# jinhan/tacotron2-vae

Hardware: AMD Instinct MI355X
Metric: mel-frames/s (train step, batch=6, 80-mel) (higher is better)
Workload: dtype f32; 1 GPU; configs[1]: Tacotron2-VAE fp32 train step (fwd+loss+bwd+clip+Adam), B=6/GPU fixed shape T_in=84 T_out=400, dropout on, random-init seed 1234; step_mode=hip-graph replay, decoder_forward=persistent, decoder_backward=persistent, startup_steps=43, global_batch=6, parallelism=dp1

## Files before the change

include/t2vae.h:

```cpp
#ifndef T2VAE_H
#define T2VAE_H
#include <stdint.h>
#ifdef __cplusplus
extern "C" {
#endif

#define T2V_OK 0
#define T2V_ERR_DIMS -1
#define T2V_ERR_ARG -2
#define T2V_ERR_LAUNCH -3

const char* t2v_version(void);
const char* t2v_last_error(void);

void t2v_set_phase_profile(unsigned long long* dev_buf32);
int t2v_stamp(unsigned long long* dev_buf, int slot, void* stream);
int t2v_debug_spin(int wgs, int microseconds, void* stream);

typedef struct t2v_step_params {
    uint64_t epoch;
    float lr;
    float bc1;
    float bc2s;
    float kl_weight;
// ... 224 lines not shown
int t2v_decoder_infer_steps_window(const t2v_dec_weights* w, const t2v_dec_infer_bufs* s, int B, int T_in,
                                   int t_begin, int t_end, float gate_threshold, float p_prenet,
                                   int external_prenet, uint64_t seed, const t2v_dec_items* items,
                                   const t2v_dec_window* window, void* stream);
int t2v_decoder_infer_persistent_window(const t2v_dec_persist_weights* w, const t2v_dec_persist_bufs* s, int B, int T_in,
                                        int t_end, float gate_threshold, float p_prenet, uint64_t seed,
                                        const t2v_dec_items* items, const t2v_dec_window* window, void* stream);

int t2v_decoder_infer_steps_plan(const t2v_dec_weights* w, const t2v_dec_infer_bufs* s, int B, int T_in,
                                 int t_begin, int t_end, float gate_threshold, float p_prenet,
                                 int external_prenet, uint64_t seed, const t2v_dec_items* items,
                                 const t2v_dec_window* window, const int32_t* plan, int plan_stride, const int32_t* n_plan,
                                 void* stream);
int t2v_decoder_infer_persistent_plan(const t2v_dec_persist_weights* w, const t2v_dec_persist_bufs* s, int B, int T_in,
                                      int t_end, float gate_threshold, float p_prenet, uint64_t seed,
                                      const t2v_dec_items* items, const t2v_dec_window* window, const int32_t* plan,
                                      int plan_stride, const int32_t* n_plan, void* stream);

#define T2V_PLAN_MAX_SYMBOLS 4096
int t2v_duration_plan(const float* dur, int dur_stride, const int32_t* n_ids, const float* rate, int rate_stride_b,
                      int rate_stride_j, int B, int S, int T_max, int32_t* plan, int plan_stride, int32_t* n_plan,
                      void* stream);

int t2v_conv1d_stat_blocks(int B, int T, int Cin, int Cout, int KS);
int t2v_conv1d_stat_blocks_bf16(int B, int T, int Cin, int Cout, int KS);
long long t2v_conv1d_staged_launches(void);
int t2v_conv1d_fwd(const float* W, const float* X, const float* bias, float* Y, float* stat_part,
                   int B, int Cin, int T, int Cout, int KS, void* stream);
int t2v_conv1d_dw_scratch_floats(int B, int Cin, int T, int Cout, int KS);
int t2v_conv1d_bwd(const float* W, const float* X, const float* dY, float* dX, float* dW, float* Wt_scratch,
                   float* dw_scratch,
                   int B, int Cin, int T, int Cout, int KS, void* stream);
int t2v_conv1d_flip_weights(const float* const* W, float* const* Wt, const int* Cout, const int* Cin, int KS, int n,
                            void* stream);
int t2v_conv1d_fwd_bf16(const float* W, const float* X, const float* bias, float* Y, float* stat_part,
                        void* Wp_scratch, int B, int Cin, int T, int Cout, int KS, void* stream);
int t2v_conv1d_bwd_bf16(const float* W, const float* X, const float* dY, float* dX, float* dW,
                        void* Wp_scratch, float* dw_scratch, int B, int Cin, int T, int Cout, int KS, void* stream);

int t2v_bn_act_fwd(const float* y, const float* stat_part, int nblk, const float* gamma, const float* beta,
                   float* running_mean, float* running_var, float* mean_out, float* rstd_out, float* out,
                   int B, int M, int T, int act, int training, float p_drop, float momentum, float eps,
                   uint64_t seed, uint32_t rng_stream, uint32_t rng_t, void* stream);
int t2v_bn_act_fwd_len(const float* y, const float* gamma, const float* beta, const float* running_mean,
                       const float* running_var, float* out, const int32_t* lengths, int B, int M, int T, int act, float eps,
                       void* stream);
int t2v_bn_act_bwd(const float* y, const float* dout, const float* mean, const float* rstd,
                   const float* gamma, const float* beta, float* dy, float* dgamma, float* dbeta,
                   float* dconv_bias, int B, int M, int T, int act, float p_drop, uint64_t seed,
                   uint32_t rng_stream, uint32_t rng_t, void* stream);
int t2v_bn_act_bwd_eval(const float* y, const float* dout, const float* mean, const float* rstd,
                   const float* gamma, const float* beta, float* dy, float* dgamma, float* dbeta,
                   float* dconv_bias, int B, int M, int T, int act, float p_drop, uint64_t seed,
                   uint32_t rng_stream, uint32_t rng_t, void* stream);
int t2v_bn_act_slices(int backward, int B, int M, int T, int training, int has_partials);

int t2v_embedding_fwd(const long long* ids, const float* W, float* out_bct, int B, int T, int C, int n_symbols, void* stream);
int t2v_embedding_bwd(const long long* ids, const float* dy_bct, float* dW, int B, int T, int C, int n_symbols, void* stream);

int t2v_gemm_epilogue_bwd(const float* dy, const float* y, float* out, size_t n, float scale, void* stream);

long t2v_colsum_scratch_floats(long M, long N);
int t2v_colsum(const float* A, long lda, long M, long N, float* scratch, float* out, void* stream);

int t2v_mask_outputs(float* mel, float* mel_post, float* gate, const int* lengths, int B, int C, int T, float gate_fill,
                     void* stream);
int t2v_mask_time(const float* x, float* out, const int32_t* lengths, int B, int C, int T, void* stream);
int t2v_reparam_fwd(const float* eps, const float* mu, const float* logvar, float* z, long n, void* stream);
int t2v_reparam_bwd(const float* dz, const float* eps, const float* logvar, float* dlogvar, long n, void* stream);
int t2v_gather_words(const void* const* src, void* const* dst, int n, void* stream);
int t2v_concat2_rows(const float* a, long lda, int na, const float* b, long ldb, int nb, float* out, long rows, void* stream);

int t2v_bilstm_fwd(const float* gx, const float* whh, const int32_t* lengths, float* y, float* gates,
                   float* cells, float* hx_scratch, uint32_t* sync3, int B, int T, void* stream);
int t2v_bilstm_bwd(const float* whh, const int32_t* lengths, const float* dy, const float* gates,
                   const float* cells, float* dg, float* dgx_scratch, uint32_t* sync3, int B, int T,
                   void* stream);

int t2v_gemm_f32(const float* A, long sAi, long sAk, const float* B, long sBj, long sBk, const float* bias,
                 float* C, int ldc, int M, int N, int K, int relu, int accumulate, float p_drop,
                 uint64_t seed, uint32_t rng_stream, uint32_t rng_t, void* stream);
long t2v_gemm_splitk_scratch_floats(int M, int N, int K);
int t2v_gemm_f32_splitk(const float* A, long sAi, long sAk, const float* B, long sBj, long sBk, const float* bias,
                        float* C, int ldc, int M, int N, int K, int relu, int accumulate, float p_drop,
                        uint64_t seed, uint32_t rng_stream, uint32_t rng_t, float* splitk_scratch, void* stream);

int t2v_gemm_f32_set_mode(int x3);

typedef struct t2v_gemm_group {
    const float* A;
    long sAi;
    long sAk;
    int nb;
    const float* B[3];
    long sBj[3];
    long sBk[3];
    int N[3];
    float* C[3];
    int ldc[3];
} t2v_gemm_group;
long t2v_gemm_f32_grouped_scratch_floats(const t2v_gemm_group* groups, int ngroups, int M, int K);
int t2v_gemm_f32_grouped(const t2v_gemm_group* groups, int ngroups, int M, int K, int accumulate, float* scratch, void* stream);
long t2v_gemm_f32_grouped_group_offset(const t2v_gemm_group* groups, int ngroups, int M, int K, int g);
int t2v_gemm_f32_grouped_handed(const t2v_gemm_group* groups, int ngroups, int M, int K, int accumulate, float* scratch, int handed,
                                const uint32_t* done_ctr, int done_cap, void* stream);
long t2v_gemm_bf16_grouped_scratch_floats(const t2v_gemm_group* groups, int ngroups, int M, int K);
int t2v_gemm_bf16_grouped(const t2v_gemm_group* groups, int ngroups, int M, int K, int accumulate, float* scratch, void* stream);

int t2v_conv1d_x3_set_mode(int mode);
int t2v_conv1d_takes_x3(int B, int Cin, int T, int Cout, int KS, int bf16);
#define T2V_CONV_OP_FWD 0
#define T2V_CONV_OP_DX 1
#define T2V_CONV_OP_DW 2
#define T2V_CONV_ROUTE_GEMM 0
#define T2V_CONV_ROUTE_FWD 1
#define T2V_CONV_ROUTE_FWD_DMA 2
#define T2V_CONV_ROUTE_X3 3
#define T2V_CONV_ROUTE_BF16 4
#define T2V_CONV_ROUTE_BF16K32 5
#define T2V_CONV_ROUTE_PLANE1 6
#define T2V_CONV_ROUTE_DW 7
#define T2V_CONV_ROUTE_DW_BF16 8
#define T2V_CONV_ROUTES 9
int t2v_conv1d_route(int op, int B, int Cin, int T, int Cout, int KS, int bf16, int w_mod16, int* fallback, int* tile, int* ksplit,
                     int* dw_splits, int* stat_blocks, int* dw_scratch_floats, int* plane_splits, int* plane_chunk);
const char* t2v_conv1d_route_name(int route);

int t2v_gemm_f32_batched(const float* A, long sAb, long sAi, long sAk, const float* B, long sBb, long sBj, long sBk,
                         float* C, long sCb, int ldc, int nbatch, int M, int N, int K, void* stream);
int t2v_gemm_bf16(const float* A, long sAi, long sAk, const float* B, long sBj, long sBk, const float* bias,
                  float* C, int ldc, int M, int N, int K, int relu, int accumulate, float p_drop,
                  uint64_t seed, uint32_t rng_stream, uint32_t rng_t, void* stream);
long t2v_gemm_bf16_splitk_scratch_floats(int M, int N, int K);
int t2v_gemm_bf16_splitk(const float* A, long sAi, long sAk, const float* B, long sBj, long sBk, const float* bias,
                         float* C, int ldc, int M, int N, int K, int relu, int accumulate, float p_drop,
                         uint64_t seed, uint32_t rng_stream, uint32_t rng_t, float* splitk_scratch, void* stream);

#define T2V_GEMM_ROUTE_F32_64 0
#define T2V_GEMM_ROUTE_F32_64_SPLITK 1
#define T2V_GEMM_ROUTE_F32_BIG_128 2
#define T2V_GEMM_ROUTE_F32_BIG_64 3
#define T2V_GEMM_ROUTE_F32_X3 4
#define T2V_GEMM_ROUTE_BF16_64 5
#define T2V_GEMM_ROUTE_BF16_64_SPLITK 6
#define T2V_GEMM_ROUTE_BF16_BIG 7
#define T2V_GEMM_ROUTE_BF16_BIG_SPLITK 8
#define T2V_GEMM_ROUTE_BF16_PLANES 9
#define T2V_GEMM_ROUTE_BF16_TO_F32_BIG 10
#define T2V_GEMM_ROUTES 11
int t2v_gemm_route(int M, int N, int K, long sAi, long sAk, long sBj, long sBk, int a_mod16, int b_mod16, int scratch_mod16,
                   int has_scratch, int relu, float p_drop, int bf16, int* form, int* splits, int* k_per_split);
const char* t2v_gemm_route_name(int route);


int t2v_conv2d_s2_fwd(const float* x, const float* w, const float* bias, float* y, int B, int Cx, int H, int W,
                      int Cout, int coord, void* stream);
int t2v_conv2d_s2_dw_scratch_floats(int B, int Cx, int H, int W, int Cout, int coord);
int t2v_conv2d_s2_bwd(const float* x, const float* w, const float* dy, float* dx, float* dw, float* dw_scratch,
                      int B, int Cx, int H, int W, int Cout, int coord, void* stream);

long t2v_conv2d_s2_gemm_scratch_floats(int B, int Cx, int H, int W, int Cout, int coord);
int t2v_conv2d_s2_fwd_gemm(const float* x, const float* w, const float* bias, float* y, float* scratch, int B, int Cx, int H, int W,
                           int Cout, int coord, void* stream);
int t2v_conv2d_s2_bwd_gemm(const float* x, const float* w, const float* dy, float* dx, float* dw, float* scratch, int B, int Cx, int H,
                           int W, int Cout, int coord, void* stream);
int t2v_gru_fwd(const float* gi, const float* whh, const float* bhh, float* hs, float* gsave, float* xchg,
                uint32_t* sync2, int B, int T, void* stream);
int t2v_gru_bwd(const float* whh, const float* hs, const float* gsave, const float* dh_last, float* dgi,
                float* dgh, float* xchg, uint32_t* sync2, int B, int T, void* stream);

int t2v_conv2d_s2_fwd_ragged(const float* x, const float* w, const float* bias, float* y, const int32_t* hlen, int B, int Cx,
                             int H, int W, int Cout, int coord, int x_tstride, void* stream);
long t2v_conv2d_s2_gemm_ragged_scratch_floats(int B, int Cx, int H, int W, int Cout, int coord);
int t2v_conv2d_s2_fwd_gemm_ragged(const float* x, const float* w, const float* bias, float* y, float* scratch,
                                  const int32_t* hlen, int B, int Cx, int H, int W, int Cout, int coord, int x_tstride,
                                  void* stream);
int t2v_gru_fwd_len(const float* gi, const float* whh, const float* bhh, float* hs, float* gsave, float* xchg,
                    uint32_t* sync2, const int32_t* steps, float* h_last, int B, int T, void* stream);
int t2v_loss_fwd_bwd(const float* mel, const float* post, const float* mel_t, const float* gate,
                     const float* gate_t, const float* mu, const float* logvar, float* dmel, float* dpost,
                     float* dgate, float* dmu, float* dlogvar, float* part192, float* out4, uint32_t* ticket,
                     uint64_t n_mel, int n_gate, int n_lat, float kl_weight, void* stream);

int t2v_clip_adam_step(float* params, float* grads, float* exp_avg, float* exp_avg_sq, uint64_t n,
                       float lr, float beta1, float beta2, float eps, float weight_decay,
                       float max_norm, float inv_world, float bc1, float bc2, float* partials,
                       float* norm_out, void* stream);
int t2v_clip_adam_step_guarded(float* params, float* grads, float* exp_avg, float* exp_avg_sq, uint64_t n,
                               float lr, float beta1, float beta2, float eps, float weight_decay,
                               float max_norm, float inv_world, float bc1, float bc2, float* partials,
                               float* norm_out, const uint32_t* guard, int guard_n, void* stream);
int t2v_clip_adam_ema_step_guarded(float* params, float* grads, float* exp_avg, float* exp_avg_sq, uint64_t n,
                                   float lr, float beta1, float beta2, float eps, float weight_decay,
                                   float max_norm, float inv_world, float bc1, float bc2, float* partials,
                                   float* norm_out, const uint32_t* guard, int guard_n, float* ema, float ema_rate,
                                   int ema_warmup, uint64_t ema_t, void* stream);

int t2v_mel_frontend(const float* wav_f32, const int16_t* wav_i16, const int64_t* n_samples, int B,
                     int n_stride, float scale, int n_fft, int hop, int n_mel, const float* window,
                     const float* tw512, const float* tw1024, const int32_t* mel_start,
                     const int32_t* mel_len, const float* mel_w, int maxw, float* mel_out,
                     int t_stride, void* stream);

int t2v_stft_polar(const float* wav, const int64_t* n_samples, int B, int n_stride, int n_fft, int hop,
                   const float* window, const float* tw512, const float* tw1024, float* mag, float* phase,
                   int t_stride, void* stream);
size_t t2v_istft_scratch_bytes(int B, int t_stride);
int t2v_istft(const float* mag, const float* phase, const int32_t* n_frames, int B, int t_stride, int n_fft, int hop,
              const float* window, const float* tw512, const float* tw1024, void* scratch, float* out, int out_stride,
              void* stream);
size_t t2v_griffin_lim_scratch_bytes(int B, int t_stride);
int t2v_griffin_lim(const float* mag, const float* angles, const int32_t* n_frames, int B, int t_stride, int n_fft,
                    int hop, int n_iters, const float* window, const float* tw512, const float* tw1024, void* scratch,
                    float* out, int out_stride, void* stream);
int t2v_mel_to_magnitude(const float* mel, const float* pinv_basis, const int32_t* n_frames, int B, int t_stride,
                         int n_mel, float* mag, void* stream);
size_t t2v_griffin_lim_fast_scratch_bytes(int B, int t_stride);
int t2v_griffin_lim_fast(const float* mag, const float* angles, const int32_t* n_frames, int B, int t_stride, int n_fft,
                         int hop, int n_iters, float momentum, const float* window, const float* tw512,
                         const float* tw1024, void* scratch, float* out, int out_stride, void* stream);
int t2v_mel_to_magnitude_nnls(const float* mel, const float* pinv_basis, const int32_t* tap_lo, const float* tap_w0,
                              const float* tap_w1, const int32_t* filt_start, const int32_t* filt_len, float lipschitz,
                              int n_iters, const int32_t* n_frames, int B, int t_stride, int n_mel, float* mag,
                              void* stream);

#define T2V_DTW_MAX_FRAMES 2048
size_t t2v_mel_dtw_scratch_bytes(int B, int tx_max, int ty_max);
int t2v_mel_dtw(const float* X, const int32_t* nx, int x_stride, const float* Y, const int32_t* ny, int y_stride,
                int B, int n_mel, float* dist, void* scratch, void* stream);

#define T2V_TSNE_MAX_POINTS 16384
#define T2V_TSNE_EXAG_ITERS 250
size_t t2v_tsne_scratch_bytes(int N, int D);
int t2v_tsne_affinities(const float* X, int N, int D, float perplexity, float* P, void* scratch, void* stream);
int t2v_tsne_gradient(const float* P, const float* Y, int N, float exaggeration, float* grad, float* kl_or_null,
                      void* scratch, void* stream);
int t2v_tsne_run(const float* P, float* Y_inout, int N, int n_iter, float learning_rate, float* kl_trace, void* scratch,
                 void* stream);

#define T2V_F0_MAX_LAG 400
int t2v_f0_yin(const float* y, const int32_t* n, int y_stride, int B, int tau_min, int tau_max, float threshold, float* f0,
               float* aperiodicity, int out_stride, void* stream);

#define T2V_ALIGN_FRAMES 16
size_t t2v_alignment_scratch_bytes(int B, int N, int T_in);
int t2v_alignment_stats(const float* A, long long a_stride_b, long long a_stride_t, const int32_t* n_frames,
                        const int32_t* n_text, int B, int N, int T_in, int max_jump, float cover_min, int32_t* path,
                        int path_stride, float* mass, int mass_stride, float* focus, int32_t* stats, void* scratch,
                        void* stream);

#define T2V_RESAMPLE_MAX_TAPS 32768
int t2v_resample(const void* x, int x_is_pcm16, float scale, const int32_t* n, int x_stride, int B, const float* taps, int up,
                 int down, int half, float* y, int out_stride, void* stream);
int t2v_trim_bounds(const float* y, const int32_t* n, int y_stride, int B, float top_db, int pad_frames, float* ms, int ms_stride,
                    int32_t* bounds, void* stream);
int t2v_crop_rows(const float* y, int y_stride, const int32_t* bounds, int B, void* out, int out_is_pcm16, int out_stride,
                  int32_t* stats, void* stream);

#define T2V_LATENT_MAX_POINTS 16384
#define T2V_LATENT_MAX_CLASSES 8
#define T2V_LATENT_MAX_K 32
#define T2V_LATENT_TILE 128
size_t t2v_latent_scratch_bytes(int N, int M, int C, int k, int slice_rows);
int t2v_latent_neighbours(const float* R, const int32_t* labels, int N, int D, int C, const float* Q, int M,
                          const int32_t* exclude, const int32_t* target, int k, int slice_rows, int32_t* nn_idx,
                          float* nn_dist, float* class_sum, int32_t* class_cnt, int32_t* rank, void* scratch, void* stream);

#define T2V_NCEP 13
#define T2V_ALIGNED_COUNTS 4
#define T2V_ALIGNED_SUMS 8
int t2v_mel_cepstrum(const float* M, const int32_t* n, int m_stride, int B, int n_mel, int n_cep, const float* table, float* out,
                     int out_stride, void* stream);
size_t t2v_cep_dtw_scratch_bytes(int B, int tx_max, int ty_max);
int t2v_cep_dtw_forward(const float* X, const int32_t* nx, int x_stride, const float* Y, const int32_t* ny, int y_stride, int B,
                        int n_cep, float* dist, void* scratch, void* stream);
int t2v_cep_dtw_walk(const int32_t* nx, int x_stride, const int32_t* ny, int y_stride, int B, const void* scratch, int32_t* K,
                     int32_t* path, int path_stride, void* stream);
int t2v_cep_dtw_path(const float* X, const int32_t* nx, int x_stride, const float* Y, const int32_t* ny, int y_stride, int B,
                     int n_cep, float* dist, int32_t* K, int32_t* path, int path_stride, void* scratch, void* stream);
int t2v_path_scores(const int32_t* path, const int32_t* K, int path_stride, const float* X, const int32_t* nx, int x_stride,
                    const float* Y, const int32_t* ny, int y_stride, const float* fx, int fx_stride, const float* fy, int fy_stride,
                    int B, int n_cep, int32_t* counts, float* sums, void* stream);

#define T2V_LOUDNESS_CHUNK 64
#define T2V_LOUDNESS_TILE 16384
size_t t2v_loudness_scratch_bytes(int B, int y_stride, int hop);
int t2v_loudness(const float* y, const int32_t* n, int y_stride, int B, const double* table, int hop, float* frame_ms,
                 int ms_stride, float* block_pw, int blk_stride, int32_t* rows, void* scratch, void* stream);
int t2v_scale_rows(float* y, const int32_t* n, int y_stride, int B, const float* gains, void* stream);

#define T2V_TSM_BINS 513
#define T2V_TSM_MAX_RATIO 1023
#define T2V_TSM_MAX_FRAMES (1 << 20)
size_t t2v_phase_vocoder_scratch_bytes(int B, int out_stride, int phase_lock);
int t2v_phase_vocoder(const float* mag, const float* phase, const int32_t* n_frames, int B, int T, int t_stride, int num, int den,
                      int phase_lock, float* mag_out, float* phase_out, int out_stride, void* scratch, void* stream);

size_t t2v_spsi_scratch_bytes(int B, int t_stride);
int t2v_spsi(const float* mag, const int32_t* n_frames, int B, int T, int t_stride, float* phase_out, void* scratch, void* stream);

#define T2V_ENV_BINS 513
#define T2V_ENV_MAX_ORDER 256
#define T2V_ENV_MAX_ITERS 32
int t2v_spectral_envelope(const float* mag, const int32_t* n_frames, int B, int T, int t_stride, int order, int iters, int p, int q,
                          float* log_env_out, float* mag_out, int out_stride, void* stream);

// ... 25 lines not shown
```

tacotron2-vae_amd/csrc/gemm.hip:

```cpp
#include <stdlib.h>
#include <string.h>
#include "t2v_common.h"
#include "t2v_kernels.h"
#include "t2v_coop.h"
#include "t2v_x3.h"
#include "t2v_xchg.h"
#include "gemm_x3_tile.h"

#define GM_BM 64
#define GM_BN 64
#define GM_BK 32

struct GemmArgs {
    const float* A; const float* B; const float* bias; float* C;
    long sAi, sAk, sBj, sBk;
    int M, N, K, ldc;
    int relu, accumulate;
    float p_drop; uint64_t seed; uint32_t rng_stream, rng_t;
    const t2v_step_params* step;
    int kz_chunk;
    float* part;
    int nbatch;
    long sAb, sBb, sCb;
    int nsub;
    long sAs, sBs;
    int bias_row;
    unsigned* tile_ctr;
};

__device__ __forceinline__ void gemm64_epilogue(const GemmArgs& a, f32x16& acc, int i0, int j0, int wm, int wn, int lane, int tid) {
    const int j = j0 + 32 * wn + (lane & 31);
    if (a.part) {
        if (j < a.N) {
#pragma unroll
            for (int r = 0; r < 16; ++r) {
                const int i = i0 + 32 * wm + (r & 3) + 8 * (r >> 2) + 4 * (lane >> 5);
                if (i < a.M) st_sc1(a.part + ((size_t)blockIdx.z * a.M + i) * a.N + j, acc[r]);
            }
        }
        __shared__ unsigned last_;
        asm volatile("s_waitcnt vmcnt(0)" ::: "memory");
        __syncthreads();
        unsigned* ctr = a.tile_ctr + blockIdx.y * gridDim.x + blockIdx.x;
        if (tid == 0) last_ = __hip_atomic_fetch_add(ctr, 1u, __ATOMIC_RELAXED, __HIP_MEMORY_SCOPE_AGENT) == gridDim.z - 1 ? 1u : 0u;
        __syncthreads();
        if (!last_) return;
        if (tid == 0) __hip_atomic_store(ctr, 0u, __ATOMIC_RELAXED, __HIP_MEMORY_SCOPE_AGENT);
        const int nz = (int)gridDim.z;
#pragma unroll
        for (int r = 0; r < 16; ++r) acc[r] = 0.f;
        if (j < a.N) {
            for (int z0 = 0; z0 < nz; z0 += 4) {
                float v[4][16];
#pragma unroll
                for (int u = 0; u < 4; ++u) {
                    const int z = min(z0 + u, nz - 1);
#pragma unroll
                    for (int r = 0; r < 16; ++r) {
                        const int i = min(i0 + 32 * wm + (r & 3) + 8 * (r >> 2) + 4 * (lane >> 5), a.M - 1);
                        v[u][r] = ld_sc1(a.part + ((size_t)z * a.M + i) * a.N + j);
                    }
                }
#pragma unroll
                for (int u = 0; u < 4; ++u)
                    if (z0 + u < nz) {
#pragma unroll
                        for (int r = 0; r < 16; ++r) acc[r] += v[u][r];
                    }
            }
        }
    }
    if (j < a.N) {
        const float bv = (a.bias && !a.bias_row) ? a.bias[j] : 0.f;
#pragma unroll
        for (int r = 0; r < 16; ++r) {
            const int i = i0 + 32 * wm + (r & 3) + 8 * (r >> 2) + 4 * (lane >> 5);
            if (i < a.M) {
                const size_t idx = (size_t)i * a.ldc + j;
                float v = acc[r] + ((a.bias && a.bias_row) ? a.bias[i] : bv);
                if (a.accumulate) v += a.C[idx];
                if (a.relu) v = fmaxf(v, 0.f);
                if (a.p_drop > 0.f) v *= t2v_drop_scale(t2v_step_seed(a.seed, a.step), a.rng_stream, a.rng_t, (uint32_t)idx, a.p_drop);
                a.C[idx] = v;
            }
        }
    }
}

template <bool A_KC, bool B_KC>
__global__ __launch_bounds__(256) void k_gemm_f32(GemmArgs a) {
    __shared__ float As[2][GM_BK][GM_BM + 1];
    __shared__ float Bs[2][GM_BK][GM_BN + 1];
    const int tid = threadIdx.x, wave = tid >> 6, lane = tid & 63;
    const int wm = wave >> 1, wn = wave & 1;
    const int i0 = blockIdx.y * GM_BM, j0 = blockIdx.x * GM_BN;
    if (a.nbatch > 1) {
        const int zb = a.nsub > 1 ? blockIdx.z / a.nsub : blockIdx.z, zs = a.nsub > 1 ? blockIdx.z - zb * a.nsub : 0;
        a.A += zb * a.sAb + zs * a.sAs; a.B += zb * a.sBb + zs * a.sBs; a.C += blockIdx.z * a.sCb;
    }
    const int kbeg = a.kz_chunk ? blockIdx.z * a.kz_chunk : 0, kend = a.kz_chunk ? min(a.K, kbeg + a.kz_chunk) : a.K;
    constexpr int NE = GM_BM * GM_BK / 256;
    float ra[NE], rb[NE];
    auto load_tiles = [&](int k0) {
#pragma unroll
        for (int e8 = 0; e8 < NE; ++e8) {
            const int e = tid + 256 * e8;
            {
                const int kk = A_KC ? (e & (GM_BK - 1)) : (e >> 6);
                const int ii = A_KC ? (e >> 5) : (e & (GM_BM - 1));
                const int i = i0 + ii, k = k0 + kk;
                ra[e8] = (i < a.M && k < kend) ? a.A[(long)i * a.sAi + (long)k * a.sAk] : 0.f;
            }
            {
                const int kk = B_KC ? (e & (GM_BK - 1)) : (e >> 6);
                const int jj = B_KC ? (e >> 5) : (e & (GM_BN - 1));
                const int j = j0 + jj, k = k0 + kk;
                rb[e8] = (j < a.N && k < kend) ? a.B[(long)j * a.sBj + (long)k * a.sBk] : 0.f;
            }
        }
    };
    auto store_tiles = [&](int buf) {
#pragma unroll
        for (int e8 = 0; e8 < NE; ++e8) {
            const int e = tid + 256 * e8;
            if (A_KC) As[buf][e & (GM_BK - 1)][e >> 5] = ra[e8]; else As[buf][e >> 6][e & (GM_BM - 1)] = ra[e8];
            if (B_KC) Bs[buf][e & (GM_BK - 1)][e >> 5] = rb[e8]; else Bs[buf][e >> 6][e & (GM_BN - 1)] = rb[e8];
        }
    };
    f32x16 acc;
#pragma unroll
    for (int r = 0; r < 16; ++r) acc[r] = 0.f;
    const int nkt = (kend - kbeg + GM_BK - 1) / GM_BK;
    load_tiles(kbeg);
    store_tiles(0);
    __syncthreads();
    const int ai = 32 * wm + (lane & 31), bj = 32 * wn + (lane & 31), kh = lane >> 5;
    for (int kt = 0; kt < nkt; ++kt) {
        const int buf = kt & 1;
        if (kt + 1 < nkt) load_tiles(kbeg + (kt + 1) * GM_BK);
#pragma unroll
        for (int s = 0; s < GM_BK / 2; ++s)
            acc = __builtin_amdgcn_mfma_f32_32x32x2f32(As[buf][2 * s + kh][ai], Bs[buf][2 * s + kh][bj], acc, 0, 0, 0);
        if (kt + 1 < nkt) store_tiles(buf ^ 1);
        __syncthreads();
    }
    gemm64_epilogue(a, acc, i0, j0, wm, wn, lane, tid);
}

#include "t2v_ring.h"
#define GM_CTR_RING ((size_t)1 << 16)
unsigned* t2v_arrival_counters(int tiles) {
    static T2VRing<unsigned, GM_CTR_RING, GM_CTR_RING, true> ring;
    return ring.take((size_t)tiles);
}
static int gemm_splits(int M, int N, int K) {
    const long tiles = (long)((M + GM_BM - 1) / GM_BM) * ((N + GM_BN - 1) / GM_BN);
    static const int wide = getenv("T2V_GEMM_SPLIT_POLICY") ? atoi(getenv("T2V_GEMM_SPLIT_POLICY")) : 1;
    if (wide) {
        if (tiles > 256 || K < 8 * GM_BK) return 1;
        long ns2 = (512 + tiles - 1) / tiles;
        const long maxk2 = K / (4 * GM_BK);
        if (ns2 > maxk2) ns2 = maxk2;
        if (ns2 > 32) ns2 = 32;
        return ns2 < 2 ? 1 : (int)ns2;
    }
    if (tiles >= 256 || K < 16 * GM_BK) return 1;
    long ns = 512 / tiles;
    const long maxk = K / (8 * GM_BK);
    if (ns > maxk) ns = maxk;
    if (ns > 32) ns = 32;
    return ns < 2 ? 1 : (int)ns;
}
static bool gemm_x3_shape_ok(int M, int N, int K);
static long gemm_x3_scratch_floats(int M, int N, int K, int np);
static int gemm_x3_mode();
extern "C" long t2v_gemm_splitk_scratch_floats(int M, int N, int K) {
    if (M < 1 || N < 1 || K < 1) return 0;
    if (gemm_x3_mode() && gemm_x3_shape_ok(M, N, K)) return gemm_x3_scratch_floats(M, N, K, 3);
    const int ns = gemm_splits(M, N, K);
    return ns > 1 ? (long)ns * M * N : 0;
}

#define GB_BM 128
#define GB_BK 32
#define GB_LD 160
template <bool A_KC, bool B_KC, int BN>
__global__ __launch_bounds__(256) void k_gemm_f32_big(GemmArgs a) {
    constexpr int NY = BN / 64;
    constexpr int NA = GB_BM * GB_BK / 4 / 256;
    constexpr int NB = BN * GB_BK / 4 / 256;
    constexpr int KQ = GB_BK / 4;
    __shared__ __attribute__((aligned(16))) float As[2][GB_BK][GB_LD];
    __shared__ __attribute__((aligned(16))) float Bs[2][GB_BK][BN + 32];
    const int tid = threadIdx.x, wave = tid >> 6, lane = tid & 63;
    const int wm = wave >> 1, wn = wave & 1;
    int by_ = blockIdx.y, bx_ = blockIdx.x;
    {
        const int nb = gridDim.x * gridDim.y, bid = blockIdx.y * gridDim.x + blockIdx.x;
        const int q = nb >> 3, r = nb & 7, xcd = bid & 7, idx = bid >> 3;
        const int lin = (xcd < r ? xcd * (q + 1) : r * (q + 1) + (xcd - r) * q) + idx;
        by_ = lin / gridDim.x;
        bx_ = lin - by_ * gridDim.x;
    }
    const int i0 = by_ * GB_BM, j0 = bx_ * BN;
    float4 ra[NA], rb[NB];
    auto load_tiles = [&](int k0) {
#pragma unroll
        for (int e = 0; e < NA; ++e) {
            if (A_KC) {
                const int i = min(i0 + tid / KQ + (256 / KQ) * e, a.M - 1), k = min(k0 + 4 * (tid % KQ), a.K - 4);
                ra[e] = *(const float4*)(a.A + (long)i * a.sAi + k);
            } else {
                const int k = min(k0 + (tid >> 5) + 8 * e, a.K - 1), i = min(i0 + 4 * (tid & 31), a.M - 4);
                ra[e] = *(const float4*)(a.A + (long)k * a.sAk + i);
            }
        }
#pragma unroll
        for (int e = 0; e < NB; ++e) {
            if (B_KC) {
                const int j = min(j0 + tid / KQ + (256 / KQ) * e, a.N - 1), k = min(k0 + 4 * (tid % KQ), a.K - 4);
                rb[e] = *(const float4*)(a.B + (long)j * a.sBj + k);
            } else {
                constexpr int RQ = BN / 4;
                const int k = min(k0 + tid / RQ + (256 / RQ) * e, a.K - 1), j = min(j0 + 4 * (tid % RQ), a.N - 4);
                rb[e] = *(const float4*)(a.B + (long)k * a.sBk + j);
            }
        }
    };
    auto store_tiles = [&](int buf, int k0) {
#pragma unroll
        for (int e = 0; e < NA; ++e) {
            if (A_KC) {
                const int m = tid / KQ + (256 / KQ) * e, kk = 4 * (tid % KQ);
                const float z = k0 + kk < a.K ? 1.f : 0.f;
                As[buf][kk + 0][m] = ra[e].x * z; As[buf][kk + 1][m] = ra[e].y * z;
                As[buf][kk + 2][m] = ra[e].z * z; As[buf][kk + 3][m] = ra[e].w * z;
            } else {
                const int kk = (tid >> 5) + 8 * e;
                const float z = k0 + kk < a.K ? 1.f : 0.f;
                *(float4*)&As[buf][kk][4 * (tid & 31)] = make_float4(ra[e].x * z, ra[e].y * z, ra[e].z * z, ra[e].w * z);
            }
        }
#pragma unroll
        for (int e = 0; e < NB; ++e) {
            if (B_KC) {
                const int n = tid / KQ + (256 / KQ) * e, kk = 4 * (tid % KQ);
                const float z = k0 + kk < a.K ? 1.f : 0.f;
                Bs[buf][kk + 0][n] = rb[e].x * z; Bs[buf][kk + 1][n] = rb[e].y * z;
                Bs[buf][kk + 2][n] = rb[e].z * z; Bs[buf][kk + 3][n] = rb[e].w * z;
            } else {
                constexpr int RQ = BN / 4;
                const int kk = tid / RQ + (256 / RQ) * e;
                const float z = k0 + kk < a.K ? 1.f : 0.f;
                *(float4*)&Bs[buf][kk][4 * (tid % RQ)] = make_float4(rb[e].x * z, rb[e].y * z, rb[e].z * z, rb[e].w * z);
            }
        }
    };
    f32x16 acc[2][NY];
#pragma unroll
    for (int x = 0; x < 2; ++x)
#pragma unroll
        for (int y = 0; y < NY; ++y)
#pragma unroll
            for (int r = 0; r < 16; ++r) acc[x][y][r] = 0.f;
    const int nkt = (a.K + GB_BK - 1) / GB_BK;
    load_tiles(0);
    store_tiles(0, 0);
    __syncthreads();
    const int am = 64 * wm + (lane & 31), bn = (BN / 2) * wn + (lane & 31), kh = lane >> 5;
    for (int kt = 0; kt < nkt; ++kt) {
        const int buf = kt & 1;
        if (kt + 1 < nkt) load_tiles((kt + 1) * GB_BK);
#pragma unroll
        for (int h = 0; h < 2; ++h) {
            float av[GB_BK / 4][2], bw[GB_BK / 4][NY];
#pragma unroll
            for (int s = 0; s < GB_BK / 4; ++s) {
                const int kr = GB_BK / 2 * h + 2 * s + kh;
                av[s][0] = As[buf][kr][am];
                av[s][1] = As[buf][kr][am + 32];
#pragma unroll
                for (int y = 0; y < NY; ++y) bw[s][y] = Bs[buf][kr][bn + 32 * y];
            }
            __builtin_amdgcn_sched_barrier(0);
#pragma unroll
            for (int s = 0; s < GB_BK / 4; ++s) {
#pragma unroll
                for (int y = 0; y < NY; ++y) {
                    acc[0][y] = __builtin_amdgcn_mfma_f32_32x32x2f32(av[s][0], bw[s][y], acc[0][y], 0, 0, 0);
                    acc[1][y] = __builtin_amdgcn_mfma_f32_32x32x2f32(av[s][1], bw[s][y], acc[1][y], 0, 0, 0);
                }
            }
        }
        if (kt + 1 < nkt) store_tiles(buf ^ 1, (kt + 1) * GB_BK);
        __syncthreads();
    }
    const uint64_t seed = t2v_step_seed(a.seed, a.step);
#pragma unroll
    for (int x = 0; x < 2; ++x)
#pragma unroll
        for (int y = 0; y < NY; ++y) {
            const int j = j0 + (BN / 2) * wn + 32 * y + (lane & 31);
            if (j < a.N) {
                const float bvs = a.bias ? a.bias[j] : 0.f;
#pragma unroll
                for (int r = 0; r < 16; ++r) {
                    const int i = i0 + 64 * wm + 32 * x + (r & 3) + 8 * (r >> 2) + 4 * (lane >> 5);
                    if (i < a.M) {
                        const size_t idx = (size_t)i * a.ldc + j;
                        float v = acc[x][y][r] + bvs;
                        if (a.accumulate) v += a.C[idx];
                        if (a.relu) v = fmaxf(v, 0.f);
                        if (a.p_drop > 0.f) v *= t2v_drop_scale(seed, a.rng_stream, a.rng_t, (uint32_t)idx, a.p_drop);
                        a.C[idx] = v;
                    }
                }
            }
        }
}

static double gemm_big_waste(int M, int N, int BN) {
    const double tiles = (double)((M + GB_BM - 1) / GB_BM) * ((N + BN - 1) / BN) * (BN / 64.0);
    const double per_cu = tiles / 256.0;
    const double unit = BN / 64.0;
// ... 572 lines not shown
    a.G = G; a.bias = nullptr; a.M = M; a.relu = 0; a.accumulate = accumulate;
    a.p_drop = 0.f; a.seed = 0; a.rng_stream = 0; a.rng_t = 0; a.step = t2v_step_for(stream);
    a.st_chunk = 0; a.part = nullptr; a.tile_ctr = nullptr;
    a.done_ctr = handed >= 0 ? done_ctr : nullptr; a.done_prod = handed >= 0 ? handed : 0; a.done_cap = (unsigned)done_cap;
    if (np == 3) k_gemm_x3p<3, 2><<<dim3(a.ntiles, 1, 1), 256, 0, stream>>>(a);
    else k_gemm_x3p<1, GX_NG1><<<dim3(a.ntiles, 1, 1), 256, 0, stream>>>(a);
    return t2v_check_launch();
}
extern "C" int t2v_gemm_f32_grouped(const t2v_gemm_group* gr, int ngroups, int M, int K, int accumulate, float* scratch, void* stream_) {
    return gemm_grouped_impl(gr, ngroups, M, K, accumulate, scratch, stream_, 3);
}
extern "C" int t2v_gemm_f32_grouped_handed(const t2v_gemm_group* gr, int ngroups, int M, int K, int accumulate, float* scratch, int handed,
                                           const uint32_t* done_ctr, int done_cap, void* stream_) {
    if (handed < 0) return T2V_ERR_ARG;
    return gemm_grouped_impl(gr, ngroups, M, K, accumulate, scratch, stream_, 3, handed, done_ctr, done_cap);
}
extern "C" long t2v_gemm_f32_grouped_group_offset(const t2v_gemm_group* gr, int ngroups, int M, int K, int g) {
    if (!gr || ngroups < 1 || ngroups > 2 || g < 0 || g >= ngroups || M < 1 || K < 1 || !gemm_grouped_x3_ok(gr, ngroups, M, K, 3)) return -1;
    return g == 0 ? 0 : gemm_grouped_scratch(gr, 1, M, K, 3);
}
extern "C" int t2v_gemm_bf16_grouped(const t2v_gemm_group* gr, int ngroups, int M, int K, int accumulate, float* scratch, void* stream_) {
    return gemm_grouped_impl(gr, ngroups, M, K, accumulate, scratch, stream_, 1);
}

__global__ __launch_bounds__(256) void k_epilogue_bwd(const float4* __restrict__ dy, const float4* __restrict__ y,
                                                      float4* __restrict__ out, size_t n4, float scale) {
    const size_t i = (size_t)blockIdx.x * 256 + threadIdx.x;
    if (i >= n4) return;
    const float4 g = dy[i], v = y[i];
    float4 o;
    o.x = v.x != 0.f ? g.x * scale : 0.f; o.y = v.y != 0.f ? g.y * scale : 0.f;
    o.z = v.z != 0.f ? g.z * scale : 0.f; o.w = v.w != 0.f ? g.w * scale : 0.f;
    out[i] = o;
}
__global__ __launch_bounds__(256) void k_epilogue_bwd_tail(const float* __restrict__ dy, const float* __restrict__ y,
                                                           float* __restrict__ out, size_t lo, size_t n, float scale) {
    const size_t i = lo + threadIdx.x;
    if (i < n) out[i] = y[i] != 0.f ? dy[i] * scale : 0.f;
}

extern "C" int t2v_gemm_epilogue_bwd(const float* dy, const float* y, float* out, size_t n, float scale, void* stream_) {
    hipStream_t stream = (hipStream_t)stream_;
    if (!dy || !y || !out || n < 1) return T2V_ERR_ARG;
    if (((uintptr_t)dy | (uintptr_t)y | (uintptr_t)out) & 15) return T2V_ERR_ARG;
    const size_t n4 = n / 4;
    if (n4) k_epilogue_bwd<<<(unsigned)((n4 + 255) / 256), 256, 0, stream>>>((const float4*)dy, (const float4*)y, (float4*)out, n4, scale);
    if (n & 3) k_epilogue_bwd_tail<<<1, 256, 0, stream>>>(dy, y, out, 4 * n4, n, scale);
    return t2v_check_launch();
}

extern "C" int t2v_gemm_f32(const float* A, long sAi, long sAk, const float* B, long sBj, long sBk, const float* bias,
                            float* C, int ldc, int M, int N, int K, int relu, int accumulate, float p_drop,
                            uint64_t seed, uint32_t rng_stream, uint32_t rng_t, void* stream_);
static int gemm_bf16_impl(const float* A, long sAi, long sAk, const float* B, long sBj, long sBk, const float* bias,
                          float* C, int ldc, int M, int N, int K, int relu, int accumulate, float p_drop,
                          uint64_t seed, uint32_t rng_stream, uint32_t rng_t, float* splitk_scratch, void* stream_);
extern "C" int t2v_gemm_bf16(const float* A, long sAi, long sAk, const float* B, long sBj, long sBk, const float* bias,
                             float* C, int ldc, int M, int N, int K, int relu, int accumulate, float p_drop,
                             uint64_t seed, uint32_t rng_stream, uint32_t rng_t, void* stream_) {
    return gemm_bf16_impl(A, sAi, sAk, B, sBj, sBk, bias, C, ldc, M, N, K, relu, accumulate, p_drop, seed, rng_stream, rng_t, nullptr, stream_);
}
extern "C" int t2v_gemm_bf16_splitk(const float* A, long sAi, long sAk, const float* B, long sBj, long sBk, const float* bias,
                                    float* C, int ldc, int M, int N, int K, int relu, int accumulate, float p_drop,
                                    uint64_t seed, uint32_t rng_stream, uint32_t rng_t, float* splitk_scratch, void* stream_) {
    return gemm_bf16_impl(A, sAi, sAk, B, sBj, sBk, bias, C, ldc, M, N, K, relu, accumulate, p_drop, seed, rng_stream, rng_t, splitk_scratch, stream_);
}
static int gemm_bf16_impl(const float* A, long sAi, long sAk, const float* B, long sBj, long sBk, const float* bias,
                          float* C, int ldc, int M, int N, int K, int relu, int accumulate, float p_drop,
                          uint64_t seed, uint32_t rng_stream, uint32_t rng_t, float* splitk_scratch, void* stream_) {
    hipStream_t stream = (hipStream_t)stream_;
    if (!A || !B || !C || M < 1 || N < 1 || K < 1 || ldc < N) return T2V_ERR_ARG;
    GemmArgs a;
    a.A = A; a.B = B; a.bias = bias; a.C = C; a.sAi = sAi; a.sAk = sAk; a.sBj = sBj; a.sBk = sBk;
    a.M = M; a.N = N; a.K = K; a.ldc = ldc; a.relu = relu; a.accumulate = accumulate;
    a.p_drop = p_drop; a.seed = seed; a.rng_stream = rng_stream; a.rng_t = rng_t; a.step = t2v_step_for(stream);
    a.kz_chunk = 0; a.part = nullptr; a.nbatch = 1; a.sAb = a.sBb = a.sCb = 0; a.nsub = 1; a.sAs = a.sBs = 0; a.bias_row = 0; a.tile_ctr = nullptr;
    const GemmRoute rt = gemm_route_bf16(gemm_shape_of(a, splitk_scratch));
    if (rt.route == T2V_GEMM_ROUTE_BF16_PLANES) return gemm_x3_run(a, splitk_scratch, stream, rt, 1);
    if (rt.route == T2V_GEMM_ROUTE_BF16_TO_F32_BIG)
        return t2v_gemm_f32(A, sAi, sAk, B, sBj, sBk, bias, C, ldc, M, N, K, relu, accumulate, p_drop, seed, rng_stream, rng_t, stream_);
    const bool big = rt.route == T2V_GEMM_ROUTE_BF16_BIG || rt.route == T2V_GEMM_ROUTE_BF16_BIG_SPLITK;
    const int bm = big ? GBB_BM : GM_BM, bn = big ? GBB_BN : GM_BN;
    dim3 grid((N + bn - 1) / bn, (M + bm - 1) / bm, rt.splits);
    if (rt.splits > 1) {
        a.kz_chunk = rt.chunk;
        a.part = splitk_scratch;
        a.tile_ctr = t2v_arrival_counters((int)(grid.x * grid.y));
        if (!a.tile_ctr) return T2V_ERR_LAUNCH;
    }
    const bool akc = rt.form & 1, bkc = (rt.form & 2) != 0;
    if (big) {
        if (akc && bkc) k_gemm_bf16_big_rr<true, true><<<grid, 256, 0, stream>>>(a);
        else if (akc) k_gemm_bf16_big_rr<true, false><<<grid, 256, 0, stream>>>(a);
        else if (bkc) k_gemm_bf16_big_rr<false, true><<<grid, 256, 0, stream>>>(a);
        else k_gemm_bf16_big_rr<false, false><<<grid, 256, 0, stream>>>(a);
        return t2v_check_launch();
    }
    if (akc && bkc) k_gemm_bf16<true, true><<<grid, 256, 0, stream>>>(a);
    else if (akc) k_gemm_bf16<true, false><<<grid, 256, 0, stream>>>(a);
    else if (bkc) k_gemm_bf16<false, true><<<grid, 256, 0, stream>>>(a);
    else k_gemm_bf16<false, false><<<grid, 256, 0, stream>>>(a);
    return t2v_check_launch();
}

static int gemm_f32_impl(const float* A, long sAi, long sAk, const float* B, long sBj, long sBk, const float* bias,
                         float* C, int ldc, int M, int N, int K, int relu, int accumulate, float p_drop,
                         uint64_t seed, uint32_t rng_stream, uint32_t rng_t, float* splitk_scratch, void* stream_);
extern "C" int t2v_gemm_f32(const float* A, long sAi, long sAk, const float* B, long sBj, long sBk, const float* bias,
                            float* C, int ldc, int M, int N, int K, int relu, int accumulate, float p_drop,
                            uint64_t seed, uint32_t rng_stream, uint32_t rng_t, void* stream_) {
    return gemm_f32_impl(A, sAi, sAk, B, sBj, sBk, bias, C, ldc, M, N, K, relu, accumulate, p_drop, seed, rng_stream, rng_t,
                         nullptr, stream_);
}
extern "C" int t2v_gemm_f32_splitk(const float* A, long sAi, long sAk, const float* B, long sBj, long sBk, const float* bias,
                                   float* C, int ldc, int M, int N, int K, int relu, int accumulate, float p_drop,
                                   uint64_t seed, uint32_t rng_stream, uint32_t rng_t, float* splitk_scratch, void* stream_) {
    return gemm_f32_impl(A, sAi, sAk, B, sBj, sBk, bias, C, ldc, M, N, K, relu, accumulate, p_drop, seed, rng_stream, rng_t,
                         splitk_scratch, stream_);
}
static int gemm_f32_impl(const float* A, long sAi, long sAk, const float* B, long sBj, long sBk, const float* bias,
                         float* C, int ldc, int M, int N, int K, int relu, int accumulate, float p_drop,
                         uint64_t seed, uint32_t rng_stream, uint32_t rng_t, float* splitk_scratch, void* stream_) {
    hipStream_t stream = (hipStream_t)stream_;
    if (!A || !B || !C || M < 1 || N < 1 || K < 1 || ldc < N) return T2V_ERR_ARG;
    GemmArgs a;
    a.A = A; a.B = B; a.bias = bias; a.C = C; a.sAi = sAi; a.sAk = sAk; a.sBj = sBj; a.sBk = sBk;
    a.M = M; a.N = N; a.K = K; a.ldc = ldc; a.relu = relu; a.accumulate = accumulate;
    a.p_drop = p_drop; a.seed = seed; a.rng_stream = rng_stream; a.rng_t = rng_t; a.step = t2v_step_for(stream);
    a.kz_chunk = 0; a.part = nullptr; a.nbatch = 1; a.sAb = a.sBb = a.sCb = 0; a.nsub = 1; a.sAs = a.sBs = 0; a.bias_row = 0; a.tile_ctr = nullptr;
    const GemmRoute rt = gemm_route_f32(gemm_shape_of(a, splitk_scratch));
    const bool akc = rt.form & 1, bkc = (rt.form & 2) != 0;
    if (rt.route == T2V_GEMM_ROUTE_F32_X3) return gemm_x3_run(a, splitk_scratch, stream, rt);
    if (rt.route == T2V_GEMM_ROUTE_F32_BIG_128 || rt.route == T2V_GEMM_ROUTE_F32_BIG_64) {
        const bool wide = rt.route == T2V_GEMM_ROUTE_F32_BIG_128;
        const int BN = wide ? 128 : 64;
        dim3 gb((N + BN - 1) / BN, (M + GB_BM - 1) / GB_BM);
#define T2V_BIG(AK, BK)                                                             \
        if (wide) k_gemm_f32_big<AK, BK, 128><<<gb, 256, 0, stream>>>(a);           \
        else k_gemm_f32_big<AK, BK, 64><<<gb, 256, 0, stream>>>(a)
        if (akc && bkc) { T2V_BIG(true, true); }
        else if (akc) { T2V_BIG(true, false); }
        else if (bkc) { T2V_BIG(false, true); }
        else { T2V_BIG(false, false); }
#undef T2V_BIG
        return t2v_check_launch();
    }
    dim3 grid((N + GM_BN - 1) / GM_BN, (M + GM_BM - 1) / GM_BM, rt.splits);
    if (rt.splits > 1) {
        a.kz_chunk = rt.chunk;
        a.part = splitk_scratch;
        a.tile_ctr = t2v_arrival_counters((int)(grid.x * grid.y));
        if (!a.tile_ctr) return T2V_ERR_LAUNCH;
    }
    if (akc && bkc) k_gemm_f32<true, true><<<grid, 256, 0, stream>>>(a);
    else if (akc) k_gemm_f32<true, false><<<grid, 256, 0, stream>>>(a);
    else if (bkc) k_gemm_f32<false, true><<<grid, 256, 0, stream>>>(a);
    else k_gemm_f32<false, false><<<grid, 256, 0, stream>>>(a);
    return t2v_check_launch();
}

int t2v_gemm_f32_batched_ex(const float* A, long sAb, long sAs, long sAi, long sAk, const float* B, long sBb, long sBs, long sBj, long sBk,
                            const float* bias_row, float* C, long sCb, int ldc, int nbatch, int nsub, int M, int N, int K, hipStream_t stream) {
    if (!A || !B || !C || nbatch < 1 || nsub < 1 || (long)nbatch * nsub > 65535 || M < 1 || N < 1 || K < 1 || ldc < N) return T2V_ERR_ARG;
    GemmArgs a;
    a.A = A; a.B = B; a.bias = bias_row; a.C = C; a.sAi = sAi; a.sAk = sAk; a.sBj = sBj; a.sBk = sBk;
    a.M = M; a.N = N; a.K = K; a.ldc = ldc; a.relu = 0; a.accumulate = 0;
    a.p_drop = 0.f; a.seed = 0; a.rng_stream = 0; a.rng_t = 0; a.step = t2v_step_for(stream);
    a.kz_chunk = 0; a.part = nullptr; a.nbatch = nbatch * nsub > 1 ? nbatch * nsub : 1; a.sAb = sAb; a.sBb = sBb; a.sCb = sCb;
    a.nsub = nsub; a.sAs = sAs; a.sBs = sBs; a.bias_row = bias_row ? 1 : 0; a.tile_ctr = nullptr;
    const bool akc = sAk == 1, bkc = sBk == 1;
    dim3 grid((N + GM_BN - 1) / GM_BN, (M + GM_BM - 1) / GM_BM, nbatch * nsub);
    if (akc && bkc) k_gemm_f32<true, true><<<grid, 256, 0, stream>>>(a);
    else if (akc) k_gemm_f32<true, false><<<grid, 256, 0, stream>>>(a);
    else if (bkc) k_gemm_f32<false, true><<<grid, 256, 0, stream>>>(a);
    else k_gemm_f32<false, false><<<grid, 256, 0, stream>>>(a);
    return t2v_check_launch();
}
extern "C" int t2v_gemm_f32_batched(const float* A, long sAb, long sAi, long sAk, const float* B, long sBb, long sBj, long sBk,
                                    float* C, long sCb, int ldc, int nbatch, int M, int N, int K, void* stream_) {
    return t2v_gemm_f32_batched_ex(A, sAb, 0, sAi, sAk, B, sBb, 0, sBj, sBk, nullptr, C, sCb, ldc, nbatch, 1, M, N, K, (hipStream_t)stream_);
}
```

Before: 230,800 mel-frames/s.

## Add deeper register-prefetch pipeline with buffer loads for 64x64 f32 GEMM

Adds a new k_gemm_f32_pipe kernel that keeps three k-tiles of global loads in flight in registers, overlapping them with MFMA on the LDS double buffer. It uses raw buffer loads with out-of-range offsets instead of branchy bounds checks, and 128-bit vector loads when alignment and strides allow. The path is enabled by default through an env-controlled switch, and the change also adds a clock probe and a shape log. The deeper prefetch raises register pressure and changes occupancy hints, which could offset the latency hiding gained.

```diff
diff --git a/include/t2vae.h b/include/t2vae.h
--- a/include/t2vae.h
+++ b/include/t2vae.h
@@ -400,6 +400,10 @@
                    int has_scratch, int relu, float p_drop, int bf16, int* form, int* splits, int* k_per_split);
 const char* t2v_gemm_route_name(int route);
 
+int t2v_gemm64_set_pipeline(int on);
+long long t2v_gemm64_pipelined_launches(void);
+int t2v_gemm64_set_probe(unsigned long long* clk2);
+
 
 int t2v_conv2d_s2_fwd(const float* x, const float* w, const float* bias, float* y, int B, int Cx, int H, int W,
                       int Cout, int coord, void* stream);
diff --git a/tacotron2-vae_amd/csrc/gemm.hip b/tacotron2-vae_amd/csrc/gemm.hip
--- a/tacotron2-vae_amd/csrc/gemm.hip
+++ b/tacotron2-vae_amd/csrc/gemm.hip
@@ -1,5 +1,8 @@
+#include <stdio.h>
 #include <stdlib.h>
 #include <string.h>
+#include <atomic>
+#include <type_traits>
 #include "t2v_common.h"
 #include "t2v_kernels.h"
 #include "t2v_coop.h"
@@ -87,8 +90,9 @@
     }
 }
 
+struct Gemm64Probe { unsigned long long* clk; };
 template <bool A_KC, bool B_KC>
-__global__ __launch_bounds__(256) void k_gemm_f32(GemmArgs a) {
+__global__ __launch_bounds__(256) void k_gemm_f32(GemmArgs a, Gemm64Probe probe) {
     __shared__ float As[2][GM_BK][GM_BM + 1];
     __shared__ float Bs[2][GM_BK][GM_BN + 1];
     const int tid = threadIdx.x, wave = tid >> 6, lane = tid & 63;
@@ -131,6 +135,8 @@
 #pragma unroll
     for (int r = 0; r < 16; ++r) acc[r] = 0.f;
     const int nkt = (kend - kbeg + GM_BK - 1) / GM_BK;
+    const bool probed = probe.clk && !(blockIdx.x | blockIdx.y | blockIdx.z) && tid == 0;
+    if (probed) probe.clk[0] = clock64();
     load_tiles(kbeg);
     store_tiles(0);
     __syncthreads();
@@ -144,6 +150,142 @@
         if (kt + 1 < nkt) store_tiles(buf ^ 1);
         __syncthreads();
     }
+    if (probed) probe.clk[1] = clock64();
+    gemm64_epilogue(a, acc, i0, j0, wm, wn, lane, tid);
+}
+
+#define GP_D 3
+template <bool A_KC, bool B_KC, bool A_V4, bool B_V4>
+__global__ __launch_bounds__(256, (A_V4 || B_V4) ? 3 : 2) void k_gemm_f32_pipe(GemmArgs a, Gemm64Probe probe) {
+    __shared__ float As[2][GM_BK][GM_BM + 1];
+    __shared__ float Bs[2][GM_BK][GM_BN + 1];
+    const int tid = threadIdx.x, wave = tid >> 6, lane = tid & 63;
+    const int wm = wave >> 1, wn = wave & 1;
+    const int i0 = blockIdx.y * GM_BM, j0 = blockIdx.x * GM_BN;
+    if (a.nbatch > 1) {
+        const int zb = a.nsub > 1 ? blockIdx.z / a.nsub : blockIdx.z, zs = a.nsub > 1 ? blockIdx.z - zb * a.nsub : 0;
+        a.A += zb * a.sAb + zs * a.sAs; a.B += zb * a.sBb + zs * a.sBs; a.C += blockIdx.z * a.sCb;
+    }
+    const int kbeg = a.kz_chunk ? blockIdx.z * a.kz_chunk : 0, kend = a.kz_chunk ? min(a.K, kbeg + a.kz_chunk) : a.K;
+    constexpr int NE = GM_BM * GM_BK / 256;
+    float ra[GP_D][NE], rb[GP_D][NE];
+    auto op_rt = [&](auto kc_, auto v4_) {
+        constexpr bool KC = decltype(kc_)::value, V4 = decltype(v4_)::value;
+        return V4 ? (KC ? tid >> 3 : 4 * (tid & 15)) : (KC ? tid >> 5 : tid & (GM_BM - 1));
+    };
+    auto op_kt = [&](auto kc_, auto v4_) {
+        constexpr bool KC = decltype(kc_)::value, V4 = decltype(v4_)::value;
+        return V4 ? (KC ? 4 * (tid & 7) : tid >> 4) : (KC ? tid & (GM_BK - 1) : tid >> 6);
+    };
+    using std::integral_constant;
+    const integral_constant<bool, A_KC> akc_; const integral_constant<bool, A_V4> av4_;
+    const integral_constant<bool, B_KC> bkc_; const integral_constant<bool, B_V4> bv4_;
+    const int a_rt = op_rt(akc_, av4_), a_kt = op_kt(akc_, av4_), b_rt = op_rt(bkc_, bv4_), b_kt = op_kt(bkc_, bv4_);
+    const float* const a_base = a.A + ((long)i0 * a.sAi + (long)kbeg * a.sAk);
+    const float* const b_base = a.B + ((long)j0 * a.sBj + (long)kbeg * a.sBk);
+    const unsigned a_tb = 4u * ((unsigned)a_rt * (unsigned)a.sAi + (unsigned)a_kt * (unsigned)a.sAk);
+    const unsigned b_tb = 4u * ((unsigned)b_rt * (unsigned)a.sBj + (unsigned)b_kt * (unsigned)a.sBk);
+    const int a_nr = a.M - i0 - a_rt, b_nr = a.N - j0 - b_rt;
+    auto load_op = [&](auto kc_, auto v4_, float* r, const float* base, long s_row, long s_k, int nr, int kt_, unsigned tb, int kofs) {
+        constexpr bool KC = decltype(kc_)::value, V4 = decltype(v4_)::value;
+        constexpr int NL = V4 ? 2 : NE, RS = KC ? GM_BM / NL : 0, KS = KC ? 0 : GM_BK / NL;
+        const int nk = kend - kbeg - kofs - kt_;
+        const __amdgpu_buffer_rsrc_t tile = t2v_rsrc(base + (long)kofs * s_k);
+        const unsigned step = 4u * (unsigned)(RS * s_row + KS * s_k);
+#pragma unroll
+        for (int n = 0; n < NL; ++n) {
+            const bool ok = RS * n < nr && KS * n < nk;
+            const unsigned vo = ok ? tb + (unsigned)n * step : 0x80000000u;
+            if constexpr (V4) {
+                const f32x4 q = __builtin_bit_cast(f32x4, __builtin_amdgcn_raw_buffer_load_b128(tile, (int)vo, 0, 0));
+                r[4 * n + 0] = q[0]; r[4 * n + 1] = q[1]; r[4 * n + 2] = q[2]; r[4 * n + 3] = q[3];
+            } else {
+                r[n] = __uint_as_float(__builtin_amdgcn_raw_buffer_load_b32(tile, (int)vo, 0, 0));
+            }
+        }
+    };
+    auto store_op = [&](auto kc_, auto v4_, const float* r, float (*S)[GM_BM + 1]) {
+        constexpr bool KC = decltype(kc_)::value, V4 = decltype(v4_)::value;
+        if constexpr (V4) {
+#pragma unroll
+            for (int h = 0; h < 2; ++h) {
+                const int v = tid + 256 * h;
+#pragma unroll
+                for (int c = 0; c < 4; ++c) {
+                    if (KC) S[4 * (v & 7) + c][v >> 3] = r[4 * h + c]; else S[v >> 4][4 * (v & 15) + c] = r[4 * h + c];
+                }
+            }
+        } else {
+#pragma unroll
+            for (int e8 = 0; e8 < NE; ++e8) {
+                const int e = tid + 256 * e8;
+                if (KC) S[e & (GM_BK - 1)][e >> 5] = r[e8]; else S[e >> 6][e & (GM_BM - 1)] = r[e8];
+            }
+        }
+    };
+    auto load_tiles = [&](int set, int kt) {
+        load_op(akc_, av4_, ra[set], a_base, a.sAi, a.sAk, a_nr, a_kt, a_tb, kt * GM_BK);
+        load_op(bkc_, bv4_, rb[set], b_base, a.sBj, a.sBk, b_nr, b_kt, b_tb, kt * GM_BK);
+    };
+    auto store_tiles = [&](int set, int buf) {
+        store_op(akc_, av4_, ra[set], As[buf]);
+        store_op(bkc_, bv4_, rb[set], Bs[buf]);
+    };
+    f32x16 acc;
+#pragma unroll
+    for (int r = 0; r < 16; ++r) acc[r] = 0.f;
+    const int nkt = (kend - kbeg + GM_BK - 1) / GM_BK;
+    const int ai = 32 * wm + (lane & 31), bj = 32 * wn + (lane & 31), kh = lane >> 5;
+    auto mfma_tile = [&](int buf) {
+#pragma unroll
+        for (int s = 0; s < GM_BK / 2; ++s)
+            acc = __builtin_amdgcn_mfma_f32_32x32x2f32(As[buf][2 * s + kh][ai], Bs[buf][2 * s + kh][bj], acc, 0, 0, 0);
+    };
+    auto tail = [&](auto r_, int kt) {
+        constexpr int R = decltype(r_)::value;
+#pragma unroll
+        for (int u = 0; u < R; ++u) {
+            if (u + GP_D < R) load_tiles(u % GP_D, kt + u + GP_D);
+            mfma_tile((kt + u) & 1);
+            if (u + 1 < R) store_tiles((u + 1) % GP_D, (kt + u + 1) & 1);
+            __syncthreads();
+        }
+    };
+    const bool probed = probe.clk && !(blockIdx.x | blockIdx.y | blockIdx.z) && tid == 0;
+    if (probed) probe.clk[0] = clock64();
+    if (nkt >= GP_D) {
+#pragma unroll
+        for (int u = 0; u < GP_D; ++u) load_tiles(u, u);
+        store_tiles(0, 0);
+        __syncthreads();
+        int kt = 0;
+        for (; kt + 2 * GP_D <= nkt; kt += GP_D) {
+#pragma unroll
+            for (int u = 0; u < GP_D; ++u) {
+                load_tiles(u, kt + u + GP_D);
+                mfma_tile((kt + u) & 1);
+                store_tiles((u + 1) % GP_D, (kt + u + 1) & 1);
+                __syncthreads();
+            }
+        }
+        static_assert(GP_D == 3, "one tail per count of k-tiles left: GP_D .. 2 GP_D - 1");
+        switch (nkt - kt) {
+        case 3: tail(integral_constant<int, 3>(), kt); break;
+        case 4: tail(integral_constant<int, 4>(), kt); break;
+        default: tail(integral_constant<int, 5>(), kt);
+        }
+    } else if (nkt == 2) {
+        load_tiles(0, 0); load_tiles(1, 1);
+        store_tiles(0, 0);
+        __syncthreads();
+        tail(integral_constant<int, 2>(), 0);
+    } else if (nkt == 1) {
+        load_tiles(0, 0);
+        store_tiles(0, 0);
+        __syncthreads();
+        tail(integral_constant<int, 1>(), 0);
+    }
+    if (probed) probe.clk[1] = clock64();
     gemm64_epilogue(a, acc, i0, j0, wm, wn, lane, tid);
 }
 
@@ -170,6 +312,70 @@
     if (ns > maxk) ns = maxk;
     if (ns > 32) ns = 32;
     return ns < 2 ? 1 : (int)ns;
+}
+static std::atomic<int> g_gemm64_pipeline{-1};
+static std::atomic<long long> g_gemm64_pipelined_launches{0};
+static std::atomic<unsigned long long*> g_gemm64_probe{nullptr};
+extern "C" int t2v_gemm64_set_pipeline(int on) {
+    int cur = g_gemm64_pipeline.load(std::memory_order_relaxed);
+    if (cur < 0) {
+        const char* e = getenv("T2V_GEMM64_PIPELINE");
+        cur = (e && *e) ? (atoi(e) != 0) : 1;
+        g_gemm64_pipeline.store(cur, std::memory_order_relaxed);
+    }
+    if (on >= 0) g_gemm64_pipeline.store(on != 0, std::memory_order_relaxed);
+    return cur;
+}
+extern "C" long long t2v_gemm64_pipelined_launches(void) { return g_gemm64_pipelined_launches.load(std::memory_order_relaxed); }
+extern "C" int t2v_gemm64_set_probe(unsigned long long* clk2) {
+    g_gemm64_probe.store(clk2, std::memory_order_relaxed);
+    return T2V_OK;
+}
+static bool gemm64_tile_span_ok(long s_row, long s_k) {
+    return s_row >= 0 && s_k >= 0 && s_row < (1L << 22) && s_k < (1L << 22);
+}
+static bool gemm64_pipelined(const GemmArgs& a, const dim3&) {
+    return t2v_gemm64_set_pipeline(-1) != 0 && gemm64_tile_span_ok(a.sAi, a.sAk) && gemm64_tile_span_ok(a.sBj, a.sBk);
+}
+static bool gemm64_vec4_ok(const float* P, long s_row, long s_k, int rows, int K, bool batched, long s_b, long s_s) {
+    if (((uintptr_t)P & 15) || (batched && ((s_b | s_s) & 3))) return false;
+    if (s_k == 1) return !(s_row & 3) && !(K & 3);
+    return s_row == 1 && !(s_k & 3) && !(rows & 3);
+}
+static void gemm64_log(const GemmArgs& a, const dim3& grid, bool pipe, bool av4, bool bv4) {
+    static FILE* f = getenv("T2V_GEMM64_LOG") ? fopen(getenv("T2V_GEMM64_LOG"), "a") : nullptr;
+    if (!f) return;
+    fprintf(f, "gemm64 M %d N %d K %d sAi %ld sAk %ld sBj %ld sBk %ld ldc %d nbatch %d nsub %d sAb %ld sAs %ld sBb %ld sBs %ld sCb %ld "
+               "splits %d chunk %d a_mod %d b_mod %d bias %d bias_row %d grid %u %u %u pipe %d v4 %d %d\n",
+            a.M, a.N, a.K, a.sAi, a.sAk, a.sBj, a.sBk, a.ldc, a.nbatch > 1 ? a.nbatch / a.nsub : 1, a.nsub, a.sAb, a.sAs, a.sBb, a.sBs, a.sCb,
+            a.kz_chunk ? (int)grid.z : 1, a.kz_chunk, (int)((uintptr_t)a.A & 15), (int)((uintptr_t)a.B & 15), a.bias != nullptr, a.bias_row,
+            grid.x, grid.y, grid.z, (int)pipe, (int)av4, (int)bv4);
+    fflush(f);
+}
+static int gemm64_launch(const GemmArgs& a, const dim3& grid, hipStream_t stream) {
+    const bool akc = a.sAk == 1, bkc = a.sBk == 1;
+    const Gemm64Probe probe{g_gemm64_probe.load(std::memory_order_relaxed)};
+    const bool pipe = gemm64_pipelined(a, grid);
+    const bool av4 = pipe && gemm64_vec4_ok(a.A, a.sAi, a.sAk, a.M, a.K, a.nbatch > 1, a.sAb, a.sAs);
+    const bool bv4 = pipe && gemm64_vec4_ok(a.B, a.sBj, a.sBk, a.N, a.K, a.nbatch > 1, a.sBb, a.sBs);
+    gemm64_log(a, grid, pipe, av4, bv4);
+    if (!pipe) {
+        if (akc && bkc) k_gemm_f32<true, true><<<grid, 256, 0, stream>>>(a, probe);
+        else if (akc) k_gemm_f32<true, false><<<grid, 256, 0, stream>>>(a, probe);
+        else if (bkc) k_gemm_f32<false, true><<<grid, 256, 0, stream>>>(a, probe);
+        else k_gemm_f32<false, false><<<grid, 256, 0, stream>>>(a, probe);
+        return t2v_check_launch();
+    }
+#define T2V_PIPE_B(AK, AV)                                                                                  \
+    if (bkc) { if (bv4) k_gemm_f32_pipe<AK, true, AV, true><<<grid, 256, 0, stream>>>(a, probe);            \
+               else k_gemm_f32_pipe<AK, true, AV, false><<<grid, 256, 0, stream>>>(a, probe); }             \
+    else { if (bv4) k_gemm_f32_pipe<AK, false, AV, true><<<grid, 256, 0, stream>>>(a, probe);               \
+           else k_gemm_f32_pipe<AK, false, AV, false><<<grid, 256, 0, stream>>>(a, probe); }
+    if (akc) { if (av4) { T2V_PIPE_B(true, true) } else { T2V_PIPE_B(true, false) } }
+    else { if (av4) { T2V_PIPE_B(false, true) } else { T2V_PIPE_B(false, false) } }
+#undef T2V_PIPE_B
+    g_gemm64_pipelined_launches.fetch_add(1, std::memory_order_relaxed);
+    return t2v_check_launch();
 }
 static bool gemm_x3_shape_ok(int M, int N, int K);
 static long gemm_x3_scratch_floats(int M, int N, int K, int np);
@@ -1048,11 +1254,7 @@
         a.tile_ctr = t2v_arrival_counters((int)(grid.x * grid.y));
         if (!a.tile_ctr) return T2V_ERR_LAUNCH;
     }
-    if (akc && bkc) k_gemm_f32<true, true><<<grid, 256, 0, stream>>>(a);
-    else if (akc) k_gemm_f32<true, false><<<grid, 256, 0, stream>>>(a);
-    else if (bkc) k_gemm_f32<false, true><<<grid, 256, 0, stream>>>(a);
-    else k_gemm_f32<false, false><<<grid, 256, 0, stream>>>(a);
-    return t2v_check_launch();
+    return gemm64_launch(a, grid, stream);
 }
 
 int t2v_gemm_f32_batched_ex(const float* A, long sAb, long sAs, long sAi, long sAk, const float* B, long sBb, long sBs, long sBj, long sBk,
@@ -1064,13 +1266,8 @@
     a.p_drop = 0.f; a.seed = 0; a.rng_stream = 0; a.rng_t = 0; a.step = t2v_step_for(stream);
     a.kz_chunk = 0; a.part = nullptr; a.nbatch = nbatch * nsub > 1 ? nbatch * nsub : 1; a.sAb = sAb; a.sBb = sBb; a.sCb = sCb;
     a.nsub = nsub; a.sAs = sAs; a.sBs = sBs; a.bias_row = bias_row ? 1 : 0; a.tile_ctr = nullptr;
-    const bool akc = sAk == 1, bkc = sBk == 1;
     dim3 grid((N + GM_BN - 1) / GM_BN, (M + GM_BM - 1) / GM_BM, nbatch * nsub);
-    if (akc && bkc) k_gemm_f32<true, true><<<grid, 256, 0, stream>>>(a);
-    else if (akc) k_gemm_f32<true, false><<<grid, 256, 0, stream>>>(a);
-    else if (bkc) k_gemm_f32<false, true><<<grid, 256, 0, stream>>>(a);
-    else k_gemm_f32<false, false><<<grid, 256, 0, stream>>>(a);
-    return t2v_check_launch();
+    return gemm64_launch(a, grid, stream);
 }
 extern "C" int t2v_gemm_f32_batched(const float* A, long sAb, long sAi, long sAk, const float* B, long sBb, long sBj, long sBk,
                                     float* C, long sCb, int ldc, int nbatch, int M, int N, int K, void* stream_) {
```

Result: no change. 231,800 mel-frames/s, median of 6 (+0.4%).
